# Samleo8/RadarSLAMPy

Measured on AMD Instinct MI355X. Metric: radar scan-pairs/sec (400x3768 polar), higher is better.
Workload: dtype u8/f32/f64

## Files before the change

### radarslampy_amd/csrc/engine_measure.hip

```cpp
#include "engine.h"

static const char *kStageNames[ST_COUNT] = {"ingest_peaks", "warp_quantise", "pyramid", "klt", "consistency_graph",
                                            "max_clique", "kabsch", "mds_lm", "glue", "retrack"};

enum { KN_INTEGRAL = ST_PYR + 1, KN_DET, KN_FUSED, KN_UNKNOWN };
static int kernel_of(const char *name)
{
    for (int i = 0; i <= ST_PYR; i++) if (!strcmp(name, kStageNames[i])) return i;
    if (!strcmp(name, "doh_integral")) return KN_INTEGRAL;
    if (!strcmp(name, "doh_det_maxima")) return KN_DET;
    return strncmp(name, "doh_fused", 9) ? KN_UNKNOWN : KN_FUSED;
}

static int32_t detect_slots(roam_ctx *ctx, Engine *e, int P)
{
    std::vector<int32_t> sc(P);
    for (int i = 0; i < P; i++) sc[i] = e->last_scan[i % e->B] >= 0 ? e->last_scan[i % e->B] : 0;
    HIP_TRY(ctx, hipMemcpy(e->rt.rt_scan, sc.data(), sizeof(int32_t) * (size_t)P, hipMemcpyHostToDevice));
    HIP_TRY(ctx, hipMemcpy(e->rt.rt_n, &P, sizeof(int32_t), hipMemcpyHostToDevice));
    return ROAM_OK;
}

int32_t fused_tables(roam_ctx *ctx, Engine *e)
{
    RtArgs &r = e->rt;
    if (r.fd_mapT) return ROAM_OK;
    const size_t npx = (size_t)e->W * e->W, R = (size_t)r.slots;
    uint32_t *mapT = nullptr, *boxtab = nullptr, *darktab = nullptr;
    bool ok = dalloc(ctx, e, &mapT, npx) && dalloc(ctx, e, &boxtab, retrack_fused_boxtab_words(e->W)) && dalloc(ctx, e, &darktab, retrack_darktab_words(e->W));
    ok = ok && dalloc(ctx, e, &r.fd_halo, R * 2 * (size_t)r.fd_halo_words) && dalloc(ctx, e, &r.fd_cc, R * 2048);
    if (!ok) return ROAM_E_HIP;
    HIP_TRY(ctx, launch_retrack_fused_tables(ctx->stream, e->warp_map, e->W, e->cfg.clip, mapT, boxtab, darktab));
    HIP_TRY(ctx, hipStreamSynchronize(ctx->stream));
    r.fd_boxtab = boxtab; r.fd_darktab = darktab;
    r.fd_mapT = mapT;
    return ROAM_OK;
}

extern "C" {

int32_t roam_engine_set_stage_events(roam_ctx *ctx, int32_t on)
{
    ENGINE();
    if (!e->stage_ev_forced) e->stage_ev = on != 0;
    return ROAM_OK;
}

int32_t roam_engine_stage_times(roam_ctx *ctx, float *ms_out, const char **names_out, int32_t cap, int32_t *n)
{
    ENGINE();
    ARG_CHECK(ctx, ms_out && n && cap >= ST_COUNT);
    if (!e->stepped) { ROAM_SET_ERR(ctx, "no step recorded"); return ROAM_E_STATE; }
    if (!e->stage_ev) { ROAM_SET_ERR(ctx, "stage events are off (roam_engine_set_stage_events)"); return ROAM_E_STATE; }
    if (e->stage_ev_step != e->nstep - 1) { ROAM_SET_ERR(ctx, "the last step was enqueued with stage events off: run a step first"); return ROAM_E_STATE; }
    HIP_TRY(ctx, hipStreamSynchronize(ctx->stream));
    for (int i = 0; i < ST_COUNT; i++) {
        float ms = 0;
        hipEvent_t *tl = e->tr_ev[(e->nstep - 1) & 63];
        if (i == ST_PEAKS) HIP_TRY(ctx, hipEventElapsedTime(&ms, tl[0], tl[5]));
        else if (i == ST_WARP) HIP_TRY(ctx, hipEventElapsedTime(&ms, tl[1], tl[2]));
        else if (i == ST_PYR) HIP_TRY(ctx, hipEventElapsedTime(&ms, tl[3], tl[4]));
        else HIP_TRY(ctx, hipEventElapsedTime(&ms, e->ev[i], e->ev[i + 1]));
        ms_out[i] = ms;
// ... 23 lines not shown
    double sum = 0;
    int64_t used = 0;
    for (int64_t i = e->nstep - n; i < e->nstep; i++) {
        if (!ok[i & 63]) continue;
        float ms = 0;
        HIP_TRY(ctx, hipEventElapsedTime(&ms, ring[(i & 63) * pitch + a0], ring[(i & 63) * pitch + a1]));
        sum += ms; used++;
    }
    *avg_ms = used ? (float)(sum / (double)used) : 0.f;
    *n_used = (int32_t)used;
    return ROAM_OK;
}

int32_t roam_engine_detect_chunk(roam_ctx *ctx, int32_t *chunk)
{
    ENGINE();
    ARG_CHECK(ctx, chunk);
    if (!e->rt_on) { ROAM_SET_ERR(ctx, "engine created without retrack_on_device"); return ROAM_E_STATE; }
    *chunk = e->det_chunk();
    return ROAM_OK;
}

int32_t roam_engine_kernel_chunk_ms(roam_ctx *ctx, const char *name, int32_t last_steps, float *ms_out, int32_t cap, int32_t *chunks,
                                    int32_t *steps_out)
{
    ENGINE();
    ARG_CHECK(ctx, name && last_steps >= 1 && ms_out && chunks && steps_out);
    const int kd = kernel_of(name) - KN_INTEGRAL;
    if (kd < 0 || kd > 1) { ROAM_SET_ERR(ctx, "unknown kernel '%s'", name); return ROAM_E_ARG; }
    if (!e->rt_on) { ROAM_SET_ERR(ctx, "engine created without retrack_on_device"); return ROAM_E_STATE; }
    if (!e->stepped) { ROAM_SET_ERR(ctx, "run a step first"); return ROAM_E_STATE; }
    HIP_TRY(ctx, hipStreamSynchronize(ctx->stream));
    const int64_t n = std::min<int64_t>(std::min<int64_t>(last_steps, e->nstep), 64);
    const int nchunk = std::min((e->B + e->det_chunk() - 1) / e->det_chunk(), RT_TRACE_CHUNKS);
    ARG_CHECK(ctx, (int64_t)cap >= n * nchunk);
    for (int64_t i = e->nstep - n, s = 0; i < e->nstep; i++, s++)
        for (int c = 0; c < nchunk; c++) {
            float ms = -1.f;
            if (e->rt_ev_ok[i & 63]) HIP_TRY(ctx, hipEventElapsedTime(&ms, e->rt_ev[i & 63][3 * c + kd], e->rt_ev[i & 63][3 * c + kd + 1]));
            ms_out[s * nchunk + c] = ms;
        }
    *chunks = nchunk;
    *steps_out = (int32_t)n;
    return ROAM_OK;
}

int32_t roam_engine_time_kernel(roam_ctx *ctx, const char *name, int32_t reps, float *avg_ms, double *algo_bytes)
{
    ENGINE();
    ARG_CHECK(ctx, name && reps >= 1 && avg_ms);
    if (!e->stepped) { ROAM_SET_ERR(ctx, "run a step first"); return ROAM_E_STATE; }
    const int k = kernel_of(name);
    if (k == KN_UNKNOWN) { ROAM_SET_ERR(ctx, "unknown kernel '%s'", name); return ROAM_E_ARG; }
    if (k >= KN_INTEGRAL && !e->rt_on) { ROAM_SET_ERR(ctx, "engine created without retrack_on_device"); return ROAM_E_STATE; }
    hipStream_t st = ctx->stream;
    const roam_engine_cfg &c = e->cfg;
    const int B = e->B;
    uint8_t *next = e->pyr[(e->cur + 1) & 3];
    double bytes = 0;
    hipEvent_t a, b;
    HIP_TRY(ctx, hipEventCreate(&a));
    HIP_TRY(ctx, hipEventCreate(&b));
    HIP_TRY(ctx, hipStreamSynchronize(st));
    HIP_TRY(ctx, hipEventRecord(a, st));
    for (int r = 0; r < reps; r++) {
        if (k == ST_WARP) {
            HIP_TRY(ctx, launch_warp_gather(st, e->warp_map, pool_warp_src(e, e->scan_idx[e->pk]), B, c.rows, c.clip, next, e->pd.lane_stride, e->warp_dark_zero));
            bytes = (double)B * ((double)c.rows * c.clip + (double)e->W * e->W);
        } else if (k == ST_PEAKS) {
            PeakSrc ps = {e->pool, (int64_t)e->rec_bytes, (int64_t)c.stride, c.payload_off, 1, e->scan_idx[e->pk]};
            hipError_t er = launch_peaks(st, ps, B, c.rows, c.clip, e->row_stage, e->stage_cap, e->row_count, e->peaks_out[(e->pk + 1) % 3], c.peaks_cap, e->peaks_n[(e->pk + 1) % 3]);
            HIP_TRY(ctx, er);
            bytes = (double)B * ((double)c.rows * c.clip);
        } else if (k == ST_PYR) {
            HIP_TRY(ctx, launch_build_pyramid(st, next, e->pd, B, e->pyr_dark));
            double rd = 0, wr = 0;
            for (int l = 0; l + 1 < ROAM_PYR_LEVELS; l++) { rd += (double)e->pd.w[l] * e->pd.h[l]; wr += (double)e->pd.w[l + 1] * e->pd.h[l + 1]; }
            bytes = (double)B * (rd + wr);
        } else {
            const int P = e->rt.slots, which = k < KN_FUSED ? k - KN_INTEGRAL : 2 + (name[9] == ':' ? atoi(name + 10) : 0);
            if (which >= 2) ROAM_TRY(fused_tables(ctx, e));
            if (r == 0) {
                ROAM_TRY(detect_slots(ctx, e, P));
                if (which == 1) HIP_TRY(ctx, launch_retrack_part(st, e->rt, P, 0));
                HIP_TRY(ctx, hipStreamSynchronize(st));
                HIP_TRY(ctx, hipEventRecord(a, st));
            }
            HIP_TRY(ctx, launch_retrack_part(st, e->rt, P, which));
            if (which >= 1) HIP_TRY(ctx, hipMemsetAsync(e->rt.cand_n, 0, sizeof(int32_t) * (size_t)P, st));
            const double npx = (double)e->W * e->W;
            const double ipx = e->rt_image_px > 0 ? (double)e->rt_image_px : npx;
            bytes = (double)P * (which == 0 ? ((double)c.rows * c.clip + ipx * 8.0) : (which == 1 ? ipx * 8.0 : (double)c.rows * c.clip));
        }
    }
    HIP_TRY(ctx, hipEventRecord(b, st));
    HIP_TRY(ctx, hipStreamSynchronize(st));
    float ms = 0;
    HIP_TRY(ctx, hipEventElapsedTime(&ms, a, b));
    hipEventDestroy(a); hipEventDestroy(b);
    *avg_ms = ms / reps;
    if (algo_bytes) *algo_bytes = bytes;
    return ROAM_OK;
}

int32_t roam_engine_debug_detect(roam_ctx *ctx, int32_t fused, int32_t n_slots, int32_t cap_per_slot, uint32_t *rc_out, double *val_out,
                                 int32_t *n_out, int32_t s_slot, double *S_out)
{
    ENGINE();
    ARG_CHECK(ctx, n_slots >= 1 && cap_per_slot >= 0 && n_out);
    if (!e->rt_on || !e->stepped) { ROAM_SET_ERR(ctx, "debug_detect: needs retrack_on_device and one step"); return ROAM_E_STATE; }
    ARG_CHECK(ctx, n_slots <= e->rt.slots && n_slots <= e->B && (!S_out || (s_slot >= 0 && s_slot < n_slots)));
    hipStream_t st = ctx->stream;
    const int P = n_slots;
    HIP_TRY(ctx, hipStreamSynchronize(st));
    ROAM_TRY(detect_slots(ctx, e, P));
    HIP_TRY(ctx, hipMemsetAsync(e->rt.cand_n, 0, sizeof(int32_t) * (size_t)P, st));
    if (fused) ROAM_TRY(fused_tables(ctx, e));
    if (fused) HIP_TRY(ctx, launch_retrack_part(st, e->rt, P, S_out ? 3 : 2));
    else { HIP_TRY(ctx, launch_retrack_part(st, e->rt, P, 0)); HIP_TRY(ctx, launch_retrack_part(st, e->rt, P, 1)); }
    HIP_TRY(ctx, launch_retrack_emit(st, e->rt, P));
    HIP_TRY(ctx, hipStreamSynchronize(st));
    HIP_TRY(ctx, hipMemcpy(n_out, e->rt.cand_n, sizeof(int32_t) * (size_t)P, hipMemcpyDeviceToHost));
    const int keep = std::min(cap_per_slot, BP_MAX_PTS);
    for (int i = 0; i < P && keep > 0; i++) {
        if (rc_out) HIP_TRY(ctx, hipMemcpy(rc_out + (size_t)i * cap_per_slot, e->rt.cand_rc + (size_t)i * BP_MAX_PTS, sizeof(uint32_t) * (size_t)keep, hipMemcpyDeviceToHost));
        if (val_out) HIP_TRY(ctx, hipMemcpy(val_out + (size_t)i * cap_per_slot, e->rt.cand_val + (size_t)i * BP_MAX_PTS, sizeof(double) * (size_t)keep, hipMemcpyDeviceToHost));
    }
    if (S_out)
        HIP_TRY(ctx, hipMemcpy2D(S_out, sizeof(double) * (size_t)e->W, e->rt.S + (size_t)s_slot * e->rt.SP * e->W, sizeof(double) * (size_t)e->rt.SP,
                                 sizeof(double) * (size_t)e->W, (size_t)e->W, hipMemcpyDeviceToHost));
    HIP_TRY(ctx, hipMemset(e->rt.cand_n, 0, sizeof(int32_t) * (size_t)P));
// ... 55 lines not shown
```

### radarslampy_amd/csrc/pyrklt.hip

```cpp
#include "roam_internal.h"

__device__ __forceinline__ int reflect101(int p, int len)
{
    if (len == 1) return 0;
    while (p < 0 || p >= len) {
        if (p < 0) p = -p;
        else p = 2 * len - 2 - p;
    }
    return p;
}

#define PD_TW 64
#define PD_TH 32
#define PD_IW (2 * PD_TW + 3)
#define PD_IH (2 * PD_TH + 3)
#define PD_IWP 132

#define PD_FW 136
__global__ __launch_bounds__(256) void pyr_down_kernel(const uint8_t *__restrict__ src, int64_t src_lane_stride,
                                                       int w, int h, uint8_t *__restrict__ dst,
                                                       int64_t dst_lane_stride, int dw, int dh)
{
    __shared__ __align__(16) uint8_t tin[PD_IH][PD_FW];
    __shared__ __align__(16) uint16_t hb[PD_IH][PD_TW];
// ... 508 lines not shown
    return hipGetLastError();
}

void pyr_desc_init(PyrDesc *d, int w, int h)
{
    int64_t off = 0;
    for (int l = 0; l < ROAM_PYR_LEVELS; l++) {
        d->w[l] = w; d->h[l] = h; d->off[l] = off;
        off += (((int64_t)w * h) + 255) & ~(int64_t)255;
        w = (w + 1) / 2; h = (h + 1) / 2;
    }
    d->lane_stride = off;
}

int pyr_two_level_kernel(const uint8_t *pyr, const PyrDesc &d, int l)
{
    const int w = d.w[l], h = d.h[l];
    if (!(l + 2 < ROAM_PYR_LEVELS && (w & 3) == 0 && w >= 64 && w <= PF_MAXW && (d.w[l + 1] & 1) == 0 && h >= 16 && d.h[l + 1] >= 8 &&
          (d.lane_stride & 3) == 0 && (d.off[l] & 3) == 0 && (d.off[l + 1] & 1) == 0 && (reinterpret_cast<uintptr_t>(pyr) & 3) == 0))
        return 0;
    return (w >= PG_MINW && w <= PG_MAXW) ? 2 : 1;
}

hipError_t launch_build_pyramid(hipStream_t st, uint8_t *pyr, const PyrDesc &d, int B, const unsigned long long *dark_l0, int first_level)
{
    for (int l = first_level; l + 1 < ROAM_PYR_LEVELS; l++) {
        const int w = d.w[l], h = d.h[l], dw = d.w[l + 1], dh = d.h[l + 1];
        if (l + 2 < ROAM_PYR_LEVELS && (w & 3) == 0 && w >= 64 && w <= PF_MAXW && (dw & 1) == 0 && h >= 16 && dh >= 8 &&
            (d.lane_stride & 3) == 0 && (d.off[l] & 3) == 0 && (d.off[l + 1] & 1) == 0 && (reinterpret_cast<uintptr_t>(pyr) & 3) == 0) {
            const int dw2 = d.w[l + 2], dh2 = d.h[l + 2];
            if (w >= PG_MINW && w <= PG_MAXW) {
                const int bands = (dh2 + PG_CC - 1) / PG_CC;
                hipLaunchKernelGGL(pyr_down2_wave_kernel, dim3((bands + 3) / 4, B), dim3(256), 0, st, pyr + d.off[l], d.lane_stride, w, h,
                                   pyr + d.off[l + 1], d.lane_stride, dw, dh, pyr + d.off[l + 2], d.lane_stride, dw2, dh2, bands);
            } else {
                dim3 grid((dh2 + PF_CC - 1) / PF_CC, B);
                hipLaunchKernelGGL(pyr_down2_rows_kernel, grid, dim3(256), 0, st, pyr + d.off[l], d.lane_stride, w, h,
                                   pyr + d.off[l + 1], d.lane_stride, dw, dh, pyr + d.off[l + 2], d.lane_stride, dw2, dh2);
            }
            hipError_t e = hipGetLastError();
            if (e != hipSuccess) return e;
            l++;
            continue;
        }
        hipError_t e = launch_pyr_down(st, pyr + d.off[l], d.lane_stride, w, h, pyr + d.off[l + 1], d.lane_stride, B, l == 0 ? dark_l0 : nullptr);
        if (e != hipSuccess) return e;
    }
    return hipSuccess;
}

#define KW 15
#define W_BITS 14
#define DESCALE(x, n) (((x) + (1 << ((n) - 1))) >> (n))

__device__ __forceinline__ long long wave_sum_rows_i32(int v)
{
    v += __builtin_amdgcn_update_dpp(0, v, 0xB1, 0xf, 0xf, false);
    v += __builtin_amdgcn_update_dpp(0, v, 0x4E, 0xf, 0xf, false);
    v += __builtin_amdgcn_update_dpp(0, v, 0x141, 0xf, 0xf, false);
    v += __builtin_amdgcn_update_dpp(0, v, 0x140, 0xf, 0xf, false);
    return ((long long)__builtin_amdgcn_readlane(v, 0) + (long long)__builtin_amdgcn_readlane(v, 16)) +
           ((long long)__builtin_amdgcn_readlane(v, 32) + (long long)__builtin_amdgcn_readlane(v, 48));
}

typedef uint32_t u32_a1 __attribute__((aligned(1)));

__device__ __forceinline__ void load_j_tile(const uint8_t *__restrict__ J, int w, int h, int tx0, int ty0, int lane,
                                            uint8_t (*Jt8)[36])
{
    if (tx0 >= 0 && tx0 + 32 <= w && ty0 >= 0 && ty0 + 32 <= h) {
#pragma unroll
        for (int i = lane; i < 32 * 8; i += 64) {
            const int y = i >> 3, c4 = (i & 7) * 4;
            *reinterpret_cast<uint32_t *>(&Jt8[y][c4]) = *reinterpret_cast<const u32_a1 *>(J + (int64_t)(ty0 + y) * w + (tx0 + c4));
        }
    } else {
        for (int i = lane; i < 32 * 8; i += 64) {
            const int y = i >> 3, c4 = (i & 7) * 4;
            const uint8_t *jr = J + (int64_t)reflect101(ty0 + y, h) * w;
            const uint32_t pk = (uint32_t)jr[reflect101(tx0 + c4, w)] | ((uint32_t)jr[reflect101(tx0 + c4 + 1, w)] << 8) |
                                ((uint32_t)jr[reflect101(tx0 + c4 + 2, w)] << 16) | ((uint32_t)jr[reflect101(tx0 + c4 + 3, w)] << 24);
            *reinterpret_cast<uint32_t *>(&Jt8[y][c4]) = pk;
        }
    }
}

__device__ __forceinline__ void bilin_weights(float a, float b, int &iw00, int &iw01, int &iw10, int &iw11)
{
    const float S = (float)(1 << W_BITS);
    const float na = __fsub_rn(1.f, a), nb = __fsub_rn(1.f, b);
    iw00 = __float2int_rn(__fmul_rn(__fmul_rn(na, nb), S));
    iw01 = __float2int_rn(__fmul_rn(__fmul_rn(a, nb), S));
    iw10 = __float2int_rn(__fmul_rn(__fmul_rn(na, b), S));
    iw11 = (1 << W_BITS) - iw00 - iw01 - iw10;
}

__global__ __launch_bounds__(64) void klt_kernel(const uint8_t *__restrict__ prev_pyr,
                                                 const uint8_t *__restrict__ next_pyr, PyrDesc d,
                                                 const float *__restrict__ pts, const int32_t *__restrict__ count,
                                                 int kstride, float *__restrict__ next_out,
                                                 uint8_t *__restrict__ status_out, float *__restrict__ err_out,
                                                 const float *__restrict__ guess, const float *__restrict__ lane_affine,
                                                 const uint8_t *__restrict__ lane_use)
{
    __shared__ __align__(16) uint8_t It8[18][20];
    __shared__ __align__(16) short Dx[16][20], Dy[16][20];
    __shared__ __align__(16) uint8_t Jt8[32][36];
    const int k = blockIdx.x, b = blockIdx.y, lane = threadIdx.x;
    if (count && k >= count[b]) return;
    const int64_t pidx = ((int64_t)b * kstride + k) * 2;
    const float ptx = pts[pidx], pty = pts[pidx + 1];
    const float halfWin = 7.f;
    const float FLT_SCALE = 1.f / (1 << 20);
    const float eps2 = __fmul_rn(0.03f, 0.03f);
    const float min_eig_thr = 1e-4f;
    float out_x = ptx, out_y = pty, er = 0.f;
    if (guess) { out_x = guess[pidx]; out_y = guess[pidx + 1]; }
    else if (lane_affine && (!lane_use || lane_use[b])) {
        const float *A = lane_affine + (int64_t)b * 6;
        out_x = __fadd_rn(__fadd_rn(__fmul_rn(A[0], ptx), __fmul_rn(A[1], pty)), A[2]);
        out_y = __fadd_rn(__fadd_rn(__fmul_rn(A[3], ptx), __fmul_rn(A[4], pty)), A[5]);
    }
    int st = 1;

    const int ry = lane >> 2, g4 = (lane & 3) * 4;
    int py_[4], px_[4];
    bool pv_[4];
#pragma unroll
    for (int q = 0; q < 4; q++) { py_[q] = ry; px_[q] = g4 + q; pv_[q] = (ry < KW) && (g4 + q < KW); }
    auto row5 = [&](int y, int x0, int (&out)[5]) {
        const uint32_t *rp = reinterpret_cast<const uint32_t *>(&Jt8[y][x0 & ~3]);
        const unsigned long long v = (((unsigned long long)rp[1] << 32) | rp[0]) >> (8 * (x0 & 3));
#pragma unroll
        for (int i = 0; i < 5; i++) out[i] = (int)((v >> (8 * i)) & 255ull);
    };

    for (int level = ROAM_PYR_LEVELS - 1; level >= 0; level--) {
        const int w = d.w[level], h = d.h[level];
        const uint8_t *I = prev_pyr + (int64_t)b * d.lane_stride + d.off[level];
        const uint8_t *J = next_pyr + (int64_t)b * d.lane_stride + d.off[level];
        const float scale = 1.f / (float)(1 << level);
        float px = __fmul_rn(ptx, scale), py = __fmul_rn(pty, scale);
        float nx, ny;
        if (level == ROAM_PYR_LEVELS - 1) { nx = __fmul_rn(out_x, scale); ny = __fmul_rn(out_y, scale); }
        else { nx = __fmul_rn(out_x, 2.f); ny = __fmul_rn(out_y, 2.f); }
        out_x = nx; out_y = ny;
        px = __fsub_rn(px, halfWin); py = __fsub_rn(py, halfWin);
        const int ipx = (int)floorf(px), ipy = (int)floorf(py);
        if (ipx < -KW || ipx >= w || ipy < -KW || ipy >= h) {
            if (level == 0) { st = 0; er = 0.f; }
            continue;
        }
        int iw00, iw01, iw10, iw11;
        bilin_weights(__fsub_rn(px, (float)ipx), __fsub_rn(py, (float)ipy), iw00, iw01, iw10, iw11);

        __syncthreads();
        if (ipx >= 1 && ipx + 19 <= w && ipy >= 1 && ipy + 17 <= h) {
            for (int i = lane; i < 18 * 5; i += 64) {
                const int ty = i / 5, q = i - ty * 5;
                reinterpret_cast<uint32_t *>(&It8[ty][0])[q] =
                    *reinterpret_cast<const u32_a1 *>(I + (int64_t)(ipy - 1 + ty) * w + (ipx - 1 + 4 * q));
            }
        } else {
            for (int i = lane; i < 18 * 18; i += 64) {
                int ty = i / 18, tx = i - ty * 18;
                It8[ty][tx] = I[(int64_t)reflect101(ipy - 1 + ty, h) * w + reflect101(ipx - 1 + tx, w)];
            }
        }
        __syncthreads();
        {
            const int y = lane >> 2, xg = (lane & 3) * 4;
            int tr[3][6];
#pragma unroll
            for (int rr = 0; rr < 3; rr++) {
                const uint32_t lo = *reinterpret_cast<const uint32_t *>(&It8[y + rr][xg]);
                const uint32_t hi = *reinterpret_cast<const uint32_t *>(&It8[y + rr][xg + 4]);
                tr[rr][0] = lo & 255; tr[rr][1] = (lo >> 8) & 255; tr[rr][2] = (lo >> 16) & 255; tr[rr][3] = lo >> 24;
                tr[rr][4] = hi & 255; tr[rr][5] = (hi >> 8) & 255;
            }
            short dxs[4], dys[4];
#pragma unroll
            for (int i = 0; i < 4; i++) {
                const int X = ipx + xg + i, Y = ipy + y;
                int dx = 0, dy = 0;
                if (X >= 0 && Y >= 0 && X < w && Y < h) {
                    const int a00 = tr[0][i], a01 = tr[0][i + 1], a02 = tr[0][i + 2];
                    const int a10 = tr[1][i], a12 = tr[1][i + 2];
                    const int a20 = tr[2][i], a21 = tr[2][i + 1], a22 = tr[2][i + 2];
                    dx = 3 * (a02 + a22 - a00 - a20) + 10 * (a12 - a10);
                    dy = 3 * (a20 + a22 - a00 - a02) + 10 * (a21 - a01);
                }
                dxs[i] = (short)dx; dys[i] = (short)dy;
            }
            *reinterpret_cast<uint2 *>(&Dx[y][xg]) = make_uint2((uint32_t)(uint16_t)dxs[0] | ((uint32_t)(uint16_t)dxs[1] << 16),
                                                                (uint32_t)(uint16_t)dxs[2] | ((uint32_t)(uint16_t)dxs[3] << 16));
            *reinterpret_cast<uint2 *>(&Dy[y][xg]) = make_uint2((uint32_t)(uint16_t)dys[0] | ((uint32_t)(uint16_t)dys[1] << 16),
                                                                (uint32_t)(uint16_t)dys[2] | ((uint32_t)(uint16_t)dys[3] << 16));
        }
        __syncthreads();
        int Iv[4], Ix[4], Iy[4];
        int pA11 = 0, pA12 = 0, pA22 = 0;
#pragma unroll
        for (int q = 0; q < 4; q++) { Iv[q] = 0; Ix[q] = 0; Iy[q] = 0; }
        if (ry < KW) {
            int ia[5], ib[5];
#pragma unroll
            for (int rr = 0; rr < 2; rr++) {
                const uint32_t lo = *reinterpret_cast<const uint32_t *>(&It8[ry + 1 + rr][g4]);
                const uint32_t hi = *reinterpret_cast<const uint32_t *>(&It8[ry + 1 + rr][g4 + 4]);
                int *dst = rr ? ib : ia;
                dst[0] = (lo >> 8) & 255; dst[1] = (lo >> 16) & 255; dst[2] = lo >> 24; dst[3] = hi & 255; dst[4] = (hi >> 8) & 255;
            }
            int xa[5], xb[5], ya[5], yb[5];
#pragma unroll
            for (int rr = 0; rr < 2; rr++) {
                const uint2 vx = *reinterpret_cast<const uint2 *>(&Dx[ry + rr][g4]);
                const uint2 vy = *reinterpret_cast<const uint2 *>(&Dy[ry + rr][g4]);
                const int x4 = Dx[ry + rr][g4 + 4], y4 = Dy[ry + rr][g4 + 4];
                int *dx_ = rr ? xb : xa, *dy_ = rr ? yb : ya;
                dx_[0] = (short)(vx.x & 0xffff); dx_[1] = (short)(vx.x >> 16); dx_[2] = (short)(vx.y & 0xffff); dx_[3] = (short)(vx.y >> 16); dx_[4] = x4;
                dy_[0] = (short)(vy.x & 0xffff); dy_[1] = (short)(vy.x >> 16); dy_[2] = (short)(vy.y & 0xffff); dy_[3] = (short)(vy.y >> 16); dy_[4] = y4;
            }
#pragma unroll
            for (int q = 0; q < 4; q++)
                if (pv_[q]) {
                    Iv[q] = DESCALE(__mul24(ia[q], iw00) + __mul24(ia[q + 1], iw01) + __mul24(ib[q], iw10) + __mul24(ib[q + 1], iw11), W_BITS - 5);
                    Ix[q] = DESCALE(__mul24(xa[q], iw00) + __mul24(xa[q + 1], iw01) + __mul24(xb[q], iw10) + __mul24(xb[q + 1], iw11), W_BITS);
                    Iy[q] = DESCALE(__mul24(ya[q], iw00) + __mul24(ya[q + 1], iw01) + __mul24(yb[q], iw10) + __mul24(yb[q + 1], iw11), W_BITS);
                    pA11 += __mul24(Ix[q], Ix[q]);
                    pA12 += __mul24(Ix[q], Iy[q]);
                    pA22 += __mul24(Iy[q], Iy[q]);
                }
        }
        const long long sA11 = wave_sum_rows_i32(pA11), sA12 = wave_sum_rows_i32(pA12), sA22 = wave_sum_rows_i32(pA22);
        const float A11 = __fmul_rn(__ll2float_rn(sA11), FLT_SCALE);
        const float A12 = __fmul_rn(__ll2float_rn(sA12), FLT_SCALE);
        const float A22 = __fmul_rn(__ll2float_rn(sA22), FLT_SCALE);
        float D = __fsub_rn(__fmul_rn(A11, A22), __fmul_rn(A12, A12));
        const float dA = __fsub_rn(A11, A22);
        const float minEig = __fdiv_rn(
            __fsub_rn(__fadd_rn(A22, A11),
                      rn_sqrtf(__fadd_rn(__fmul_rn(dA, dA), __fmul_rn(__fmul_rn(4.f, A12), A12)))),
            (float)(2 * KW * KW));
        if (minEig < min_eig_thr || D < 1.1920929e-07f) {
            if (level == 0) st = 0;
            continue;
        }
        D = __fdiv_rn(1.f, D);
        nx = __fsub_rn(nx, halfWin); ny = __fsub_rn(ny, halfWin);
        float pdx = 0.f, pdy = 0.f;
        int tx0 = -(1 << 28), ty0 = -(1 << 28);
        for (int j = 0; j < 10; j++) {
            const int inx = (int)floorf(nx), iny = (int)floorf(ny);
            if (inx < -KW || inx >= w || iny < -KW || iny >= h) {
                if (level == 0) st = 0;
                break;
            }
            bilin_weights(__fsub_rn(nx, (float)inx), __fsub_rn(ny, (float)iny), iw00, iw01, iw10, iw11);
            if (!(inx >= tx0 && inx - tx0 <= 15 && iny >= ty0 && iny - ty0 <= 15)) {
                tx0 = inx - 8; ty0 = iny - 8;
                __syncthreads();
                load_j_tile(J, w, h, tx0, ty0, lane, Jt8);
                __syncthreads();
            }
            const int jox = inx - tx0, joy = iny - ty0;
            int pb1 = 0, pb2 = 0;
            if (ry < KW) {
                int ra[5], rb[5];
                row5(joy + ry, jox + g4, ra);
                row5(joy + ry + 1, jox + g4, rb);
#pragma unroll
                for (int q = 0; q < 4; q++)
                    if (pv_[q]) {
                        int jv = DESCALE(__mul24(ra[q], iw00) + __mul24(ra[q + 1], iw01) + __mul24(rb[q], iw10) + __mul24(rb[q + 1], iw11), W_BITS - 5);
                        int diff = jv - Iv[q];
                        pb1 += __mul24(diff, Ix[q]);
                        pb2 += __mul24(diff, Iy[q]);
                    }
            }
            const long long sb1 = wave_sum_rows_i32(pb1), sb2 = wave_sum_rows_i32(pb2);
            const float b1 = __fmul_rn(__ll2float_rn(sb1), FLT_SCALE);
            const float b2 = __fmul_rn(__ll2float_rn(sb2), FLT_SCALE);
            const float ddx = __fmul_rn(__fsub_rn(__fmul_rn(A12, b2), __fmul_rn(A22, b1)), D);
            const float ddy = __fmul_rn(__fsub_rn(__fmul_rn(A12, b1), __fmul_rn(A11, b2)), D);
            nx = __fadd_rn(nx, ddx); ny = __fadd_rn(ny, ddy);
            out_x = __fadd_rn(nx, halfWin); out_y = __fadd_rn(ny, halfWin);
            if (__fadd_rn(__fmul_rn(ddx, ddx), __fmul_rn(ddy, ddy)) <= eps2) break;
            if (j > 0 && fabsf(__fadd_rn(ddx, pdx)) < 0.01f && fabsf(__fadd_rn(ddy, pdy)) < 0.01f) {
                out_x = __fsub_rn(out_x, __fmul_rn(ddx, 0.5f));
                out_y = __fsub_rn(out_y, __fmul_rn(ddy, 0.5f));
                break;
            }
            pdx = ddx; pdy = ddy;
        }
        if (st && level == 0) {
            const float ex = __fsub_rn(out_x, halfWin), ey = __fsub_rn(out_y, halfWin);
            const int iex = (int)floorf(ex), iey = (int)floorf(ey);
            if (iex < -KW || iex >= w || iey < -KW || iey >= h) { st = 0; continue; }
            bilin_weights(__fsub_rn(ex, (float)iex), __fsub_rn(ey, (float)iey), iw00, iw01, iw10, iw11);
            if (!(iex >= tx0 && iex - tx0 <= 15 && iey >= ty0 && iey - ty0 <= 15)) {
                tx0 = iex - 8; ty0 = iey - 8;
                __syncthreads();
                load_j_tile(J, w, h, tx0, ty0, lane, Jt8);
                __syncthreads();
            }
            const int eox = iex - tx0, eoy = iey - ty0;
            int pe = 0;
            if (ry < KW) {
                int ra[5], rb[5];
                row5(eoy + ry, eox + g4, ra);
                row5(eoy + ry + 1, eox + g4, rb);
#pragma unroll
                for (int q = 0; q < 4; q++)
                    if (pv_[q]) {
                        int jv = DESCALE(__mul24(ra[q], iw00) + __mul24(ra[q + 1], iw01) + __mul24(rb[q], iw10) + __mul24(rb[q + 1], iw11), W_BITS - 5);
                        int diff = jv - Iv[q];
                        pe += diff < 0 ? -diff : diff;
                    }
            }
            const long long se = wave_sum_rows_i32(pe);
            er = __fmul_rn(__ll2float_rn(se), 1.f / (float)(32 * KW * KW));
        }
    }
    if (lane == 0) {
        next_out[pidx] = out_x; next_out[pidx + 1] = out_y;
        status_out[(int64_t)b * kstride + k] = (uint8_t)st;
        err_out[(int64_t)b * kstride + k] = er;
    }
}

hipError_t launch_klt(hipStream_t st, const uint8_t *prev_pyr, const uint8_t *next_pyr,
                      const PyrDesc &d, const float *pts, const int32_t *count, int K, int kstride,
                      int B, float *next, uint8_t *status, float *err, const float *guess, const float *lane_affine,
                      const uint8_t *lane_use)
{
    if (K <= 0 || B <= 0) return hipSuccess;
    hipLaunchKernelGGL(klt_kernel, dim3(K, B), dim3(64), 0, st, prev_pyr, next_pyr, d, pts, count, kstride,
                       next, status, err, guess, lane_affine, lane_use);
    return hipGetLastError();
}
```

Before: 59440.

## Pack multiple KLT features per wavefront with segmented DPP reductions

```diff
diff --git a/profiles/time_klt.py b/profiles/time_klt.py
--- /dev/null
+++ b/profiles/time_klt.py
@@ -0,0 +1,48 @@
+#!/usr/bin/env python3
+import os, sys
+sys.path.insert(0, os.path.dirname(os.path.dirname(os.path.abspath(__file__))))
+import numpy as np
+import bench
+from radarslampy_amd import _ffi
+if os.environ.get("ROAM_LIB"):
+    _ffi.LIB_PATH = os.path.abspath(os.environ["ROAM_LIB"])
+from radarslampy_amd.engine import Engine
+
+LANES = [int(x) for x in (sys.argv[1] if len(sys.argv) > 1 else "4096,64").split(",")]
+T, DISTINCT, PREROLL, REPS, REPEATS = 7, 8, 16, 20, 5
+
+
+def main():
+    seqs = bench.render_sequences([17 * d + 5 for d in range(DISTINCT)], T, True, bench.WORK_RETRACK, min(DISTINCT, 8))
+    period = 2 * T - 2
+    cyc = np.array(list(range(T)) + list(range(T - 2, 0, -1)))
+    ctx = _ffi.Context(0)
+    for B in LANES:
+        eng = Engine(B, B * T, ctx=ctx, retrack_on_device=True)
+        Dn = min(DISTINCT, B)
+        for d in range(Dn):
+            for t in range(T):
+                eng.upload_scan(d * T + t, seqs[d][0][t])
+        for b in range(Dn, B):
+            for t in range(T):
+                eng.copy_scan(b * T + t, (b % Dn) * T + t)
+        eng.synchronize()
+        phase = np.array([(b // Dn) % period for b in range(B)])
+        t0 = cyc[phase]
+        eng.init_lanes_detect(0, [b * T + int(t0[b]) for b in range(B)], np.array([seqs[b % Dn][1][int(t0[b])] for b in range(B)]))
+        for i in range(PREROLL):
+            ph = (phase + i + 1) % period
+            eng.step(((np.arange(B) * T + cyc[ph]) | np.where(ph == 0, _ffi.STEP_NEW_SEQUENCE, 0)).astype(np.int32))
+        eng.synchronize()
+        counts = np.array([len(eng.lane_features(b)) for b in range(0, B, max(1, B // 64))])
+        eng.time_kernel("klt", 3)
+        ms = [eng.time_kernel("klt", REPS)[0] for _ in range(REPEATS)]
+        print(f"klt {os.path.basename(_ffi.LIB_PATH)} lanes {B}: " + " ".join(f"{m:.3f}" for m in ms) +
+              f" ms per launch ({REPS} launches each); median {np.median(ms):.3f}, spread {max(ms) - min(ms):.3f}; "
+              f"features per lane (every {max(1, B // 64)}th): mean {counts.mean():.0f}, max {counts.max()}", flush=True)
+        eng.close()
+    ctx.close()
+
+
+if __name__ == "__main__":
+    main()
diff --git a/radarslampy_amd/csrc/engine_measure.hip b/radarslampy_amd/csrc/engine_measure.hip
--- a/radarslampy_amd/csrc/engine_measure.hip
+++ b/radarslampy_amd/csrc/engine_measure.hip
@@ -3,12 +3,13 @@
 static const char *kStageNames[ST_COUNT] = {"ingest_peaks", "warp_quantise", "pyramid", "klt", "consistency_graph",
                                             "max_clique", "kabsch", "mds_lm", "glue", "retrack"};
 
-enum { KN_INTEGRAL = ST_PYR + 1, KN_DET, KN_FUSED, KN_UNKNOWN };
+enum { KN_INTEGRAL = ST_PYR + 1, KN_DET, KN_FUSED, KN_KLT, KN_UNKNOWN };
 static int kernel_of(const char *name)
 {
     for (int i = 0; i <= ST_PYR; i++) if (!strcmp(name, kStageNames[i])) return i;
     if (!strcmp(name, "doh_integral")) return KN_INTEGRAL;
     if (!strcmp(name, "doh_det_maxima")) return KN_DET;
+    if (!strcmp(name, kStageNames[ST_KLT])) return KN_KLT;
     return strncmp(name, "doh_fused", 9) ? KN_UNKNOWN : KN_FUSED;
 }
 
@@ -138,7 +139,7 @@
     if (!e->stepped) { ROAM_SET_ERR(ctx, "run a step first"); return ROAM_E_STATE; }
     const int k = kernel_of(name);
     if (k == KN_UNKNOWN) { ROAM_SET_ERR(ctx, "unknown kernel '%s'", name); return ROAM_E_ARG; }
-    if (k >= KN_INTEGRAL && !e->rt_on) { ROAM_SET_ERR(ctx, "engine created without retrack_on_device"); return ROAM_E_STATE; }
+    if (k >= KN_INTEGRAL && k != KN_KLT && !e->rt_on) { ROAM_SET_ERR(ctx, "engine created without retrack_on_device"); return ROAM_E_STATE; }
     hipStream_t st = ctx->stream;
     const roam_engine_cfg &c = e->cfg;
     const int B = e->B;
@@ -163,6 +164,9 @@
             double rd = 0, wr = 0;
             for (int l = 0; l + 1 < ROAM_PYR_LEVELS; l++) { rd += (double)e->pd.w[l] * e->pd.h[l]; wr += (double)e->pd.w[l + 1] * e->pd.h[l + 1]; }
             bytes = (double)B * (rd + wr);
+        } else if (k == KN_KLT) {
+            HIP_TRY(ctx, launch_klt(st, e->pyr[e->cur], e->pyr[(e->cur + 3) & 3], e->pd, e->feat, e->feat_n, e->kmax(), KS, B, e->klt_next,
+                                    e->klt_status, e->klt_err, nullptr, nullptr, nullptr));
         } else {
             const int P = e->rt.slots, which = k < KN_FUSED ? k - KN_INTEGRAL : 2 + (name[9] == ':' ? atoi(name + 10) : 0);
             if (which >= 2) ROAM_TRY(fused_tables(ctx, e));
diff --git a/radarslampy_amd/csrc/pyrklt.hip b/radarslampy_amd/csrc/pyrklt.hip
--- a/radarslampy_amd/csrc/pyrklt.hip
+++ b/radarslampy_amd/csrc/pyrklt.hip
@@ -584,30 +584,60 @@
 #define KW 15
 #define W_BITS 14
 #define DESCALE(x, n) (((x) + (1 << ((n) - 1))) >> (n))
-
-__device__ __forceinline__ long long wave_sum_rows_i32(int v)
+#ifndef KLT_G
+#define KLT_G 4
+#endif
+static_assert(KLT_G == 2 || KLT_G == 4, "a feature owns 32 or 16 lanes");
+
+template <int F>
+__device__ __forceinline__ int seg_sum_i32(int v)
 {
     v += __builtin_amdgcn_update_dpp(0, v, 0xB1, 0xf, 0xf, false);
     v += __builtin_amdgcn_update_dpp(0, v, 0x4E, 0xf, 0xf, false);
     v += __builtin_amdgcn_update_dpp(0, v, 0x141, 0xf, 0xf, false);
     v += __builtin_amdgcn_update_dpp(0, v, 0x140, 0xf, 0xf, false);
-    return ((long long)__builtin_amdgcn_readlane(v, 0) + (long long)__builtin_amdgcn_readlane(v, 16)) +
-           ((long long)__builtin_amdgcn_readlane(v, 32) + (long long)__builtin_amdgcn_readlane(v, 48));
+    if (F == 32) v += __shfl_xor(v, 16);
+    return v;
+}
+template <int F>
+__device__ __forceinline__ float seg_sum_u32_f32(int p)
+{
+    return __uint2float_rn((unsigned)seg_sum_i32<F>(p));
+}
+template <int F>
+__device__ __forceinline__ float seg_sum_f32(int p)
+{
+    const int lo = seg_sum_i32<F>(p & 0xffff), hi = seg_sum_i32<F>(p >> 16);
+    return __fmaf_rn((float)hi, 65536.f, (float)lo);
 }
 
 typedef uint32_t u32_a1 __attribute__((aligned(1)));
 
-__device__ __forceinline__ void load_j_tile(const uint8_t *__restrict__ J, int w, int h, int tx0, int ty0, int lane,
+struct KltSetup {
+    uint8_t It8[18][20];
+    short Dx[16][20], Dy[16][20];
+};
+struct KltTiles {
+    union {
+        KltSetup s;
+        uint8_t Jt8[32][36];
+    };
+    uint8_t pad[88];
+};
+static_assert(sizeof(KltSetup) == 1640 && sizeof(KltTiles) == 1728, "feature stride = 16 banks modulo 32");
+
+template <int F>
+__device__ __forceinline__ void load_j_tile(const uint8_t *__restrict__ J, int w, int h, int tx0, int ty0, int fl,
                                             uint8_t (*Jt8)[36])
 {
     if (tx0 >= 0 && tx0 + 32 <= w && ty0 >= 0 && ty0 + 32 <= h) {
 #pragma unroll
-        for (int i = lane; i < 32 * 8; i += 64) {
-            const int y = i >> 3, c4 = (i & 7) * 4;
+        for (int p = 0; p < 32 * 8 / F; p++) {
+            const int i = p * F + fl, y = i >> 3, c4 = (i & 7) * 4;
             *reinterpret_cast<uint32_t *>(&Jt8[y][c4]) = *reinterpret_cast<const u32_a1 *>(J + (int64_t)(ty0 + y) * w + (tx0 + c4));
         }
     } else {
-        for (int i = lane; i < 32 * 8; i += 64) {
+        for (int i = fl; i < 32 * 8; i += F) {
             const int y = i >> 3, c4 = (i & 7) * 4;
             const uint8_t *jr = J + (int64_t)reflect101(ty0 + y, h) * w;
             const uint32_t pk = (uint32_t)jr[reflect101(tx0 + c4, w)] | ((uint32_t)jr[reflect101(tx0 + c4 + 1, w)] << 8) |
@@ -615,6 +645,36 @@
             *reinterpret_cast<uint32_t *>(&Jt8[y][c4]) = pk;
         }
     }
+}
+
+template <int N, int NB>
+__device__ __forceinline__ void row_bytes(const uint8_t *row, int x0, int (&out)[NB])
+{
+    static_assert(NB <= N + 4, "bytes beyond the dwords read");
+    const uint32_t *rp = reinterpret_cast<const uint32_t *>(row + (x0 & ~3));
+    uint32_t dw[N / 4 + 1];
+#pragma unroll
+    for (int i = 0; i <= N / 4; i++) dw[i] = rp[i];
+    const int sh = 8 * (x0 & 3);
+#pragma unroll
+    for (int i = 0; 4 * i < NB; i++) {
+        const uint32_t v = i < N / 4 ? (uint32_t)(((((unsigned long long)dw[i < N / 4 ? i + 1 : i]) << 32) | dw[i]) >> sh) : dw[i] >> sh;
+#pragma unroll
+        for (int c = 0; c < 4; c++)
+            if (4 * i + c < NB) out[4 * i + c] = (int)((v >> (8 * c)) & 255u);
+    }
+}
+
+template <int N>
+__device__ __forceinline__ void row_shorts(const short *row, int x0, int (&out)[N + 1])
+{
+#pragma unroll
+    for (int i = 0; i < N / 4; i++) {
+        const uint2 v = *reinterpret_cast<const uint2 *>(row + x0 + 4 * i);
+        out[4 * i] = (short)(v.x & 0xffff); out[4 * i + 1] = (short)(v.x >> 16);
+        out[4 * i + 2] = (short)(v.y & 0xffff); out[4 * i + 3] = (short)(v.y >> 16);
+    }
+    out[N] = row[x0 + N];
 }
 
 __device__ __forceinline__ void bilin_weights(float a, float b, int &iw00, int &iw01, int &iw10, int &iw11)
@@ -629,25 +689,27 @@
 
 __global__ __launch_bounds__(64) void klt_kernel(const uint8_t *__restrict__ prev_pyr,
                                                  const uint8_t *__restrict__ next_pyr, PyrDesc d,
-                                                 const float *__restrict__ pts, const int32_t *__restrict__ count,
+                                                 const float *__restrict__ pts, const int32_t *__restrict__ count, int K,
                                                  int kstride, float *__restrict__ next_out,
                                                  uint8_t *__restrict__ status_out, float *__restrict__ err_out,
                                                  const float *__restrict__ guess, const float *__restrict__ lane_affine,
                                                  const uint8_t *__restrict__ lane_use)
 {
-    __shared__ __align__(16) uint8_t It8[18][20];
-    __shared__ __align__(16) short Dx[16][20], Dy[16][20];
-    __shared__ __align__(16) uint8_t Jt8[32][36];
-    const int k = blockIdx.x, b = blockIdx.y, lane = threadIdx.x;
-    if (count && k >= count[b]) return;
-    const int64_t pidx = ((int64_t)b * kstride + k) * 2;
-    const float ptx = pts[pidx], pty = pts[pidx + 1];
+    constexpr int G = KLT_G, F = 64 / G, PPL = 4 * G, LPR = 4 / G;
+    __shared__ __align__(16) KltTiles tiles[G];
+    const int b = blockIdx.y, lane = threadIdx.x, fl = lane & (F - 1);
+    const int k = G * (int)blockIdx.x + lane / F;
+    const bool active = k < K && (!count || k < count[b]);
+    if (!__any(active)) return;
+    KltTiles &T = tiles[lane / F];
+    const int64_t pidx = active ? ((int64_t)b * kstride + k) * 2 : 0;
+    const float ptx = active ? pts[pidx] : 0.f, pty = active ? pts[pidx + 1] : 0.f;
     const float halfWin = 7.f;
     const float FLT_SCALE = 1.f / (1 << 20);
     const float eps2 = __fmul_rn(0.03f, 0.03f);
     const float min_eig_thr = 1e-4f;
     float out_x = ptx, out_y = pty, er = 0.f;
-    if (guess) { out_x = guess[pidx]; out_y = guess[pidx + 1]; }
+    if (guess) { if (active) { out_x = guess[pidx]; out_y = guess[pidx + 1]; } }
     else if (lane_affine && (!lane_use || lane_use[b])) {
         const float *A = lane_affine + (int64_t)b * 6;
         out_x = __fadd_rn(__fadd_rn(__fmul_rn(A[0], ptx), __fmul_rn(A[1], pty)), A[2]);
@@ -655,17 +717,11 @@
     }
     int st = 1;
 
-    const int ry = lane >> 2, g4 = (lane & 3) * 4;
-    int py_[4], px_[4];
-    bool pv_[4];
-#pragma unroll
-    for (int q = 0; q < 4; q++) { py_[q] = ry; px_[q] = g4 + q; pv_[q] = (ry < KW) && (g4 + q < KW); }
-    auto row5 = [&](int y, int x0, int (&out)[5]) {
-        const uint32_t *rp = reinterpret_cast<const uint32_t *>(&Jt8[y][x0 & ~3]);
-        const unsigned long long v = (((unsigned long long)rp[1] << 32) | rp[0]) >> (8 * (x0 & 3));
-#pragma unroll
-        for (int i = 0; i < 5; i++) out[i] = (int)((v >> (8 * i)) & 255ull);
-    };
+    const int ry = fl / LPR, g0 = (fl % LPR) * PPL;
+    const bool rowv = ry < KW;
+    bool pv_[PPL];
+#pragma unroll
+    for (int q = 0; q < PPL; q++) pv_[q] = g0 + q < KW;
 
     for (int level = ROAM_PYR_LEVELS - 1; level >= 0; level--) {
         const int w = d.w[level], h = d.h[level];
@@ -679,41 +735,39 @@
         out_x = nx; out_y = ny;
         px = __fsub_rn(px, halfWin); py = __fsub_rn(py, halfWin);
         const int ipx = (int)floorf(px), ipy = (int)floorf(py);
-        if (ipx < -KW || ipx >= w || ipy < -KW || ipy >= h) {
+        bool lv = active;
+        if (lv && (ipx < -KW || ipx >= w || ipy < -KW || ipy >= h)) {
             if (level == 0) { st = 0; er = 0.f; }
-            continue;
-        }
+            lv = false;
+        }
+        if (!__any(lv)) continue;
         int iw00, iw01, iw10, iw11;
         bilin_weights(__fsub_rn(px, (float)ipx), __fsub_rn(py, (float)ipy), iw00, iw01, iw10, iw11);
 
         __syncthreads();
-        if (ipx >= 1 && ipx + 19 <= w && ipy >= 1 && ipy + 17 <= h) {
-            for (int i = lane; i < 18 * 5; i += 64) {
-                const int ty = i / 5, q = i - ty * 5;
-                reinterpret_cast<uint32_t *>(&It8[ty][0])[q] =
-                    *reinterpret_cast<const u32_a1 *>(I + (int64_t)(ipy - 1 + ty) * w + (ipx - 1 + 4 * q));
-            }
-        } else {
-            for (int i = lane; i < 18 * 18; i += 64) {
-                int ty = i / 18, tx = i - ty * 18;
-                It8[ty][tx] = I[(int64_t)reflect101(ipy - 1 + ty, h) * w + reflect101(ipx - 1 + tx, w)];
+        if (lv) {
+            if (ipx >= 1 && ipx + 19 <= w && ipy >= 1 && ipy + 17 <= h) {
+                for (int i = fl; i < 18 * 5; i += F) {
+                    const int ty = i / 5, q = i - ty * 5;
+                    reinterpret_cast<uint32_t *>(&T.s.It8[ty][0])[q] =
+                        *reinterpret_cast<const u32_a1 *>(I + (int64_t)(ipy - 1 + ty) * w + (ipx - 1 + 4 * q));
+                }
+            } else {
+                for (int i = fl; i < 18 * 18; i += F) {
+                    int ty = i / 18, tx = i - ty * 18;
+                    T.s.It8[ty][tx] = I[(int64_t)reflect101(ipy - 1 + ty, h) * w + reflect101(ipx - 1 + tx, w)];
+                }
             }
         }
         __syncthreads();
-        {
-            const int y = lane >> 2, xg = (lane & 3) * 4;
-            int tr[3][6];
-#pragma unroll
-            for (int rr = 0; rr < 3; rr++) {
-                const uint32_t lo = *reinterpret_cast<const uint32_t *>(&It8[y + rr][xg]);
-                const uint32_t hi = *reinterpret_cast<const uint32_t *>(&It8[y + rr][xg + 4]);
-                tr[rr][0] = lo & 255; tr[rr][1] = (lo >> 8) & 255; tr[rr][2] = (lo >> 16) & 255; tr[rr][3] = lo >> 24;
-                tr[rr][4] = hi & 255; tr[rr][5] = (hi >> 8) & 255;
-            }
-            short dxs[4], dys[4];
-#pragma unroll
-            for (int i = 0; i < 4; i++) {
-                const int X = ipx + xg + i, Y = ipy + y;
+        if (lv) {
+            int tr[3][PPL + 2];
+#pragma unroll
+            for (int rr = 0; rr < 3; rr++) row_bytes<PPL, PPL + 2>(&T.s.It8[ry + rr][0], g0, tr[rr]);
+            short dxs[PPL], dys[PPL];
+#pragma unroll
+            for (int i = 0; i < PPL; i++) {
+                const int X = ipx + g0 + i, Y = ipy + ry;
                 int dx = 0, dy = 0;
                 if (X >= 0 && Y >= 0 && X < w && Y < h) {
                     const int a00 = tr[0][i], a01 = tr[0][i + 1], a02 = tr[0][i + 2];
@@ -724,37 +778,29 @@
                 }
                 dxs[i] = (short)dx; dys[i] = (short)dy;
             }
-            *reinterpret_cast<uint2 *>(&Dx[y][xg]) = make_uint2((uint32_t)(uint16_t)dxs[0] | ((uint32_t)(uint16_t)dxs[1] << 16),
-                                                                (uint32_t)(uint16_t)dxs[2] | ((uint32_t)(uint16_t)dxs[3] << 16));
-            *reinterpret_cast<uint2 *>(&Dy[y][xg]) = make_uint2((uint32_t)(uint16_t)dys[0] | ((uint32_t)(uint16_t)dys[1] << 16),
-                                                                (uint32_t)(uint16_t)dys[2] | ((uint32_t)(uint16_t)dys[3] << 16));
+#pragma unroll
+            for (int i = 0; i < PPL; i += 4) {
+                *reinterpret_cast<uint2 *>(&T.s.Dx[ry][g0 + i]) = make_uint2((uint32_t)(uint16_t)dxs[i] | ((uint32_t)(uint16_t)dxs[i + 1] << 16),
+                                                                          (uint32_t)(uint16_t)dxs[i + 2] | ((uint32_t)(uint16_t)dxs[i + 3] << 16));
+                *reinterpret_cast<uint2 *>(&T.s.Dy[ry][g0 + i]) = make_uint2((uint32_t)(uint16_t)dys[i] | ((uint32_t)(uint16_t)dys[i + 1] << 16),
+                                                                          (uint32_t)(uint16_t)dys[i + 2] | ((uint32_t)(uint16_t)dys[i + 3] << 16));
+            }
         }
         __syncthreads();
-        int Iv[4], Ix[4], Iy[4];
+        int Iv[PPL], Ix[PPL], Iy[PPL];
         int pA11 = 0, pA12 = 0, pA22 = 0;
 #pragma unroll
-        for (int q = 0; q < 4; q++) { Iv[q] = 0; Ix[q] = 0; Iy[q] = 0; }
-        if (ry < KW) {
-            int ia[5], ib[5];
-#pragma unroll
-            for (int rr = 0; rr < 2; rr++) {
-                const uint32_t lo = *reinterpret_cast<const uint32_t *>(&It8[ry + 1 + rr][g4]);
-                const uint32_t hi = *reinterpret_cast<const uint32_t *>(&It8[ry + 1 + rr][g4 + 4]);
-                int *dst = rr ? ib : ia;
-                dst[0] = (lo >> 8) & 255; dst[1] = (lo >> 16) & 255; dst[2] = lo >> 24; dst[3] = hi & 255; dst[4] = (hi >> 8) & 255;
-            }
-            int xa[5], xb[5], ya[5], yb[5];
-#pragma unroll
-            for (int rr = 0; rr < 2; rr++) {
-                const uint2 vx = *reinterpret_cast<const uint2 *>(&Dx[ry + rr][g4]);
-                const uint2 vy = *reinterpret_cast<const uint2 *>(&Dy[ry + rr][g4]);
-                const int x4 = Dx[ry + rr][g4 + 4], y4 = Dy[ry + rr][g4 + 4];
-                int *dx_ = rr ? xb : xa, *dy_ = rr ? yb : ya;
-                dx_[0] = (short)(vx.x & 0xffff); dx_[1] = (short)(vx.x >> 16); dx_[2] = (short)(vx.y & 0xffff); dx_[3] = (short)(vx.y >> 16); dx_[4] = x4;
-                dy_[0] = (short)(vy.x & 0xffff); dy_[1] = (short)(vy.x >> 16); dy_[2] = (short)(vy.y & 0xffff); dy_[3] = (short)(vy.y >> 16); dy_[4] = y4;
-            }
-#pragma unroll
-            for (int q = 0; q < 4; q++)
+        for (int q = 0; q < PPL; q++) { Iv[q] = 0; Ix[q] = 0; Iy[q] = 0; }
+        if (lv && rowv) {
+            int ia[PPL + 1], ib[PPL + 1], xa[PPL + 1], xb[PPL + 1], ya[PPL + 1], yb[PPL + 1];
+            row_bytes<PPL, PPL + 1>(&T.s.It8[ry + 1][0], g0 + 1, ia);
+            row_bytes<PPL, PPL + 1>(&T.s.It8[ry + 2][0], g0 + 1, ib);
+            row_shorts<PPL>(&T.s.Dx[ry][0], g0, xa);
+            row_shorts<PPL>(&T.s.Dx[ry + 1][0], g0, xb);
+            row_shorts<PPL>(&T.s.Dy[ry][0], g0, ya);
+            row_shorts<PPL>(&T.s.Dy[ry + 1][0], g0, yb);
+#pragma unroll
+            for (int q = 0; q < PPL; q++)
                 if (pv_[q]) {
                     Iv[q] = DESCALE(__mul24(ia[q], iw00) + __mul24(ia[q + 1], iw01) + __mul24(ib[q], iw10) + __mul24(ib[q + 1], iw11), W_BITS - 5);
                     Ix[q] = DESCALE(__mul24(xa[q], iw00) + __mul24(xa[q + 1], iw01) + __mul24(xb[q], iw10) + __mul24(xb[q + 1], iw11), W_BITS);
@@ -764,45 +810,48 @@
                     pA22 += __mul24(Iy[q], Iy[q]);
                 }
         }
-        const long long sA11 = wave_sum_rows_i32(pA11), sA12 = wave_sum_rows_i32(pA12), sA22 = wave_sum_rows_i32(pA22);
-        const float A11 = __fmul_rn(__ll2float_rn(sA11), FLT_SCALE);
-        const float A12 = __fmul_rn(__ll2float_rn(sA12), FLT_SCALE);
-        const float A22 = __fmul_rn(__ll2float_rn(sA22), FLT_SCALE);
+        const float A11 = __fmul_rn(seg_sum_u32_f32<F>(pA11), FLT_SCALE);
+        const float A12 = __fmul_rn(seg_sum_f32<F>(pA12), FLT_SCALE);
+        const float A22 = __fmul_rn(seg_sum_u32_f32<F>(pA22), FLT_SCALE);
         float D = __fsub_rn(__fmul_rn(A11, A22), __fmul_rn(A12, A12));
         const float dA = __fsub_rn(A11, A22);
         const float minEig = __fdiv_rn(
             __fsub_rn(__fadd_rn(A22, A11),
                       rn_sqrtf(__fadd_rn(__fmul_rn(dA, dA), __fmul_rn(__fmul_rn(4.f, A12), A12)))),
             (float)(2 * KW * KW));
-        if (minEig < min_eig_thr || D < 1.1920929e-07f) {
+        bool it = lv;
+        if (it && (minEig < min_eig_thr || D < 1.1920929e-07f)) {
             if (level == 0) st = 0;
-            continue;
-        }
+            it = false;
+        }
+        if (!__any(it)) continue;
         D = __fdiv_rn(1.f, D);
         nx = __fsub_rn(nx, halfWin); ny = __fsub_rn(ny, halfWin);
         float pdx = 0.f, pdy = 0.f;
         int tx0 = -(1 << 28), ty0 = -(1 << 28);
-        for (int j = 0; j < 10; j++) {
+        bool run = it;
+        for (int j = 0; j < 10 && __any(run); j++) {
             const int inx = (int)floorf(nx), iny = (int)floorf(ny);
-            if (inx < -KW || inx >= w || iny < -KW || iny >= h) {
+            if (run && (inx < -KW || inx >= w || iny < -KW || iny >= h)) {
                 if (level == 0) st = 0;
-                break;
+                run = false;
             }
             bilin_weights(__fsub_rn(nx, (float)inx), __fsub_rn(ny, (float)iny), iw00, iw01, iw10, iw11);
-            if (!(inx >= tx0 && inx - tx0 <= 15 && iny >= ty0 && iny - ty0 <= 15)) {
-                tx0 = inx - 8; ty0 = iny - 8;
+            const bool reload = run && !(inx >= tx0 && inx - tx0 <= 15 && iny >= ty0 && iny - ty0 <= 15);
+            if (__any(reload)) {
+                if (reload) { tx0 = inx - 8; ty0 = iny - 8; }
                 __syncthreads();
-                load_j_tile(J, w, h, tx0, ty0, lane, Jt8);
+                if (reload) load_j_tile<F>(J, w, h, tx0, ty0, fl, T.Jt8);
                 __syncthreads();
             }
-            const int jox = inx - tx0, joy = iny - ty0;
             int pb1 = 0, pb2 = 0;
-            if (ry < KW) {
-                int ra[5], rb[5];
-                row5(joy + ry, jox + g4, ra);
-                row5(joy + ry + 1, jox + g4, rb);
-#pragma unroll
-                for (int q = 0; q < 4; q++)
+            if (run && rowv) {
+                const int jox = inx - tx0, joy = iny - ty0;
+                int ra[PPL + 1], rb[PPL + 1];
+                row_bytes<PPL, PPL + 1>(&T.Jt8[joy + ry][0], jox + g0, ra);
+                row_bytes<PPL, PPL + 1>(&T.Jt8[joy + ry + 1][0], jox + g0, rb);
+#pragma unroll
+                for (int q = 0; q < PPL; q++)
                     if (pv_[q]) {
                         int jv = DESCALE(__mul24(ra[q], iw00) + __mul24(ra[q + 1], iw01) + __mul24(rb[q], iw10) + __mul24(rb[q + 1], iw11), W_BITS - 5);
                         int diff = jv - Iv[q];
@@ -810,51 +859,55 @@
                         pb2 += __mul24(diff, Iy[q]);
                     }
             }
-            const long long sb1 = wave_sum_rows_i32(pb1), sb2 = wave_sum_rows_i32(pb2);
-            const float b1 = __fmul_rn(__ll2float_rn(sb1), FLT_SCALE);
-            const float b2 = __fmul_rn(__ll2float_rn(sb2), FLT_SCALE);
-            const float ddx = __fmul_rn(__fsub_rn(__fmul_rn(A12, b2), __fmul_rn(A22, b1)), D);
-            const float ddy = __fmul_rn(__fsub_rn(__fmul_rn(A12, b1), __fmul_rn(A11, b2)), D);
-            nx = __fadd_rn(nx, ddx); ny = __fadd_rn(ny, ddy);
-            out_x = __fadd_rn(nx, halfWin); out_y = __fadd_rn(ny, halfWin);
-            if (__fadd_rn(__fmul_rn(ddx, ddx), __fmul_rn(ddy, ddy)) <= eps2) break;
-            if (j > 0 && fabsf(__fadd_rn(ddx, pdx)) < 0.01f && fabsf(__fadd_rn(ddy, pdy)) < 0.01f) {
-                out_x = __fsub_rn(out_x, __fmul_rn(ddx, 0.5f));
-                out_y = __fsub_rn(out_y, __fmul_rn(ddy, 0.5f));
-                break;
-            }
-            pdx = ddx; pdy = ddy;
-        }
-        if (st && level == 0) {
+            const float b1 = __fmul_rn(seg_sum_f32<F>(pb1), FLT_SCALE);
+            const float b2 = __fmul_rn(seg_sum_f32<F>(pb2), FLT_SCALE);
+            if (run) {
+                const float ddx = __fmul_rn(__fsub_rn(__fmul_rn(A12, b2), __fmul_rn(A22, b1)), D);
+                const float ddy = __fmul_rn(__fsub_rn(__fmul_rn(A12, b1), __fmul_rn(A11, b2)), D);
+                nx = __fadd_rn(nx, ddx); ny = __fadd_rn(ny, ddy);
+                out_x = __fadd_rn(nx, halfWin); out_y = __fadd_rn(ny, halfWin);
+                if (__fadd_rn(__fmul_rn(ddx, ddx), __fmul_rn(ddy, ddy)) <= eps2) run = false;
+                else if (j > 0 && fabsf(__fadd_rn(ddx, pdx)) < 0.01f && fabsf(__fadd_rn(ddy, pdy)) < 0.01f) {
+                    out_x = __fsub_rn(out_x, __fmul_rn(ddx, 0.5f));
+                    out_y = __fsub_rn(out_y, __fmul_rn(ddy, 0.5f));
+                    run = false;
+                }
+                pdx = ddx; pdy = ddy;
+            }
+        }
+        if (level == 0) {
+            bool ev = it && st;
             const float ex = __fsub_rn(out_x, halfWin), ey = __fsub_rn(out_y, halfWin);
             const int iex = (int)floorf(ex), iey = (int)floorf(ey);
-            if (iex < -KW || iex >= w || iey < -KW || iey >= h) { st = 0; continue; }
+            if (ev && (iex < -KW || iex >= w || iey < -KW || iey >= h)) { st = 0; ev = false; }
+            if (!__any(ev)) continue;
             bilin_weights(__fsub_rn(ex, (float)iex), __fsub_rn(ey, (float)iey), iw00, iw01, iw10, iw11);
-            if (!(iex >= tx0 && iex - tx0 <= 15 && iey >= ty0 && iey - ty0 <= 15)) {
-                tx0 = iex - 8; ty0 = iey - 8;
+            const bool reload = ev && !(iex >= tx0 && iex - tx0 <= 15 && iey >= ty0 && iey - ty0 <= 15);
+            if (__any(reload)) {
+                if (reload) { tx0 = iex - 8; ty0 = iey - 8; }
                 __syncthreads();
-                load_j_tile(J, w, h, tx0, ty0, lane, Jt8);
+                if (reload) load_j_tile<F>(J, w, h, tx0, ty0, fl, T.Jt8);
                 __syncthreads();
             }
-            const int eox = iex - tx0, eoy = iey - ty0;
             int pe = 0;
-            if (ry < KW) {
-                int ra[5], rb[5];
-                row5(eoy + ry, eox + g4, ra);
-                row5(eoy + ry + 1, eox + g4, rb);
-#pragma unroll
-                for (int q = 0; q < 4; q++)
+            if (ev && rowv) {
+                const int eox = iex - tx0, eoy = iey - ty0;
+                int ra[PPL + 1], rb[PPL + 1];
+                row_bytes<PPL, PPL + 1>(&T.Jt8[eoy + ry][0], eox + g0, ra);
+                row_bytes<PPL, PPL + 1>(&T.Jt8[eoy + ry + 1][0], eox + g0, rb);
+#pragma unroll
+                for (int q = 0; q < PPL; q++)
                     if (pv_[q]) {
                         int jv = DESCALE(__mul24(ra[q], iw00) + __mul24(ra[q + 1], iw01) + __mul24(rb[q], iw10) + __mul24(rb[q + 1], iw11), W_BITS - 5);
                         int diff = jv - Iv[q];
                         pe += diff < 0 ? -diff : diff;
                     }
             }
-            const long long se = wave_sum_rows_i32(pe);
-            er = __fmul_rn(__ll2float_rn(se), 1.f / (float)(32 * KW * KW));
-        }
-    }
-    if (lane == 0) {
+            const float se = seg_sum_u32_f32<F>(pe);
+            if (ev) er = __fmul_rn(se, 1.f / (float)(32 * KW * KW));
+        }
+    }
+    if (active && fl == 0) {
         next_out[pidx] = out_x; next_out[pidx + 1] = out_y;
         status_out[(int64_t)b * kstride + k] = (uint8_t)st;
         err_out[(int64_t)b * kstride + k] = er;
@@ -867,7 +920,7 @@
                       const uint8_t *lane_use)
 {
     if (K <= 0 || B <= 0) return hipSuccess;
-    hipLaunchKernelGGL(klt_kernel, dim3(K, B), dim3(64), 0, st, prev_pyr, next_pyr, d, pts, count, kstride,
+    hipLaunchKernelGGL(klt_kernel, dim3((K + KLT_G - 1) / KLT_G, B), dim3(64), 0, st, prev_pyr, next_pyr, d, pts, count, K, kstride,
                        next, status, err, guess, lane_affine, lane_use);
     return hipGetLastError();
 }
```

After: 59310. No clear change (-0.2%).
